# nicklashansen/tdmpc2

Hardware: AMD Instinct MI355X
Metric: plan() calls/sec (H=3, 512 samples, 6 iters) (higher is better)
Workload: dtype f32 (f16x2-split products: 22-bit operands, fp32 accumulate)

## Files before the change

### tdmpc2_amd/csrc/fused_kernels.cuh

```cuda
#pragma once

#include "kloop_schedule.h"

#ifdef SPLIT_TIMING
#define TIMER_FIELDS mutable unsigned long long t_acc[14] = {0, 0, 0, 0, 0, 0, 0, 0, 0, 0, 0, 0, 0, 0}; mutable unsigned long long t_last = 0, t_begin = 0;
#define TIMER_START(c) { (c).t_last = (c).t_begin = __builtin_amdgcn_s_memtime(); }
#define TIMER_MARK(c, cls) { __builtin_amdgcn_sched_barrier(0); const unsigned long long t_now = __builtin_amdgcn_s_memtime(); __builtin_amdgcn_sched_barrier(0); (c).t_acc[cls] += t_now - (c).t_last; (c).t_last = t_now; }
#ifndef SPLIT_TIMING_WAVE
#define SPLIT_TIMING_WAVE 4
#endif
#define TIMER_FLUSH(c, ptr) if ((ptr) && threadIdx.x == 64 * SPLIT_TIMING_WAVE) { for (int i_ = 0; i_ < 14; ++i_) atomicAdd((ptr) + i_, (c).t_acc[i_]); atomicAdd((ptr) + 14, (c).t_last - (c).t_begin); atomicAdd((ptr) + 15, 1ull); }
#else
#define TIMER_FIELDS
#define TIMER_START(c)
#define TIMER_MARK(c, cls)
#define TIMER_FLUSH(c, ptr)
#endif
enum { T_KLOOP = 0, T_EPI = 1, T_HEAD = 2, T_ACT = 3, T_PARK = 4, T_TILE = 5, T_EPI_PRE = 6, T_EPI_SYNC = 7, T_EPI_BIAS = 8,
       T_EPI_COMB = 9, T_EPI_MATH = 10, T_CL_WAIT = 11, T_HEAD_K = 12, T_HEAD_ST = 13 };



template <int APAD, int ST = 2, int NW = 8, int AR = 0>
struct CtxT {
    static constexpr int NST = ST;
    static constexpr int NWAVES = NW;
    static constexpr int ARITH = AR;
    static constexpr int FT = 16 / NW;
    static constexpr int NTHR = 64 * NW;
    static constexpr int TROWS = 32 * ST;
    static constexpr int SH = WIDTH + APAD;
    static constexpr int RSH = 2 * SH + 8;
    static constexpr int RSF_ = AR == 0 ? RSH / 2 : WIDTH + APAD + 4;
    static constexpr int KBLK = AR == 0 ? 16 : 8;
    static constexpr int ZKB = WIDTH / KBLK;
    _Float16 *act;
    float *stats;
    float *gb;
    int tid, wave, lane;
    mutable float pg[(WIDTH + NTHR - 1) / NTHR], pb[(WIDTH + NTHR - 1) / NTHR];
    TIMER_FIELDS
    __device__ __forceinline__ float *f32() const { return reinterpret_cast<float *>(act); }
    static constexpr __device__ __forceinline__ int RSF() { return RSF_; }
};

__device__ __forceinline__ float mish_fast(float x) {
    const float e = __expf(fminf(x, 20.f));
    const float n = e * (e + 2.f);
    return x * (n * __builtin_amdgcn_rcpf(n + 2.f));
}

template <class CT>
__device__ __forceinline__ float exp_a(float x) {
    if constexpr (CT::ARITH == 1) return expf(x);
    else return __expf(x);
}
template <class CT>
__device__ __forceinline__ float mish_a(float x) {
    if constexpr (CT::ARITH == 1) {
        const float e = expf(fminf(x, 20.f));
        const float n = e * (e + 2.f);
        return x * (n / (n + 2.f));
    } else {
        return mish_fast(x);
    }
}

__device__ __forceinline__ void split4(const f32x4 y, f16x4 &hi, f16x4 &lo, const float scale = ACT_SCALE) {
#pragma unroll
    for (int e = 0; e < 4; ++e) {
        const float ys = y[e] * scale;
        const _Float16 h = (_Float16)ys;
        hi[e] = h;
        lo[e] = (_Float16)(ys - (float)h);
    }
}


constexpr int PF = 2;
template <int FT>
struct BFragT {
    f16x8 h[FT], l[FT];
};
__device__ __forceinline__ f16x8 ldw(const char *ubase, unsigned voff, int imm) {
    return *reinterpret_cast<const f16x8 *>(ubase + voff + imm);
}
#define SPLIT_MFMA(a, b, c) __builtin_amdgcn_mfma_f32_32x32x16_f16(a, b, c, 0, 0, 0)
template <int FT>
__device__ __forceinline__ void load_b(BFragT<FT> &b, const char *u0, size_t ct_stride, unsigned voff) {
#pragma unroll
    for (int cc = 0; cc < FT; ++cc) {
        b.h[cc] = ldw(u0 + cc * ct_stride, voff, 0);
        b.l[cc] = ldw(u0 + cc * ct_stride, voff, 1024);
    }
}
template <int ST, int FT>
__device__ __forceinline__ void zero_acc(f32x16 (&a)[ST][FT]) {
#pragma unroll
    for (int r = 0; r < ST; ++r)
#pragma unroll
        for (int cc = 0; cc < FT; ++cc)
#pragma unroll
            for (int e = 0; e < 16; ++e) a[r][cc][e] = 0.f;
}
template <int ST>
struct AFragT {
    f16x8 h[ST], l[ST];
};
template <class CT>
__device__ __forceinline__ void load_a(AFragT<CT::NST> &a, const _Float16 *a0p, int kk) {
#pragma unroll
    for (int st = 0; st < CT::NST; ++st) {
        a.h[st] = *reinterpret_cast<const f16x8 *>(a0p + st * 32 * CT::RSH + kk * 16);
        a.l[st] = *reinterpret_cast<const f16x8 *>(a0p + st * 32 * CT::RSH + CT::SH + kk * 16);
    }
}
template <class CT>
__device__ __forceinline__ void kloop_f32(const CT &c, const LayerS &ly, int kb0, int kb1, f32x16 (&acc)[CT::NST][CT::FT]) {
    constexpr int FT = CT::FT, NST = CT::NST;
    constexpr int PFD = 4;
    const int i = c.lane & 31, hh = c.lane >> 5;
    const float *a0p = c.f32() + i * CT::RSF() + 4 * hh + kb0 * 8;
    const char *u0 = reinterpret_cast<const char *>(ly.wp) + ((size_t)(FT * c.wave) * ly.KB + kb0) * 1024;
    const size_t cts = (size_t)ly.KB * 1024;
    unsigned voff = (unsigned)c.lane * 16u;
    asm volatile("" : "+v"(voff));
// ... 285 lines not shown
        for (int d = 0; d < PFT; ++d) step(k + d, d, true);
    }
#pragma unroll 1
    for (; k < nk; k += PFT) {
#pragma unroll
        for (int d = 0; d < PFT; ++d)
            if (k + d < nk) step(k + d, d, false);
    }
#pragma unroll
    for (int r = 0; r < CT::NST; ++r)
#pragma unroll
        for (int e = 0; e < 16; ++e) out[r][e] = acc[r][0][e] + (acc[r][1][e] + acc[r][2][e]);
}


template <class CT>
__device__ __forceinline__ void park(const CT &c, const f32x16 (&acc)[CT::NST][CT::FT], float *dst) {
#pragma unroll
    for (int st = 0; st < CT::NST; ++st)
#pragma unroll
        for (int ft = 0; ft < CT::FT; ++ft)
#pragma unroll
            for (int m = 0; m < 4; ++m) {
                f32x4 v;
#pragma unroll
                for (int r = 0; r < 4; ++r) v[r] = acc[st][ft][4 * m + r];
                const int idx4 = ((c.wave * CT::NST + st) * CT::FT + ft) * 4 + m;
                *reinterpret_cast<f32x4 *>(dst + ((size_t)idx4 * 64 + c.lane) * 4) = v;
            }
}
template <class CT>
__device__ __forceinline__ void unpark(const CT &c, f32x16 (&acc)[CT::NST][CT::FT], const float *src) {
#pragma unroll
    for (int st = 0; st < CT::NST; ++st)
#pragma unroll
        for (int ft = 0; ft < CT::FT; ++ft)
#pragma unroll
            for (int m = 0; m < 4; ++m) {
                const int idx4 = ((c.wave * CT::NST + st) * CT::FT + ft) * 4 + m;
                const f32x4 v = *reinterpret_cast<const f32x4 *>(src + ((size_t)idx4 * 64 + c.lane) * 4);
#pragma unroll
                for (int r = 0; r < 4; ++r) acc[st][ft][4 * m + r] = v[r];
            }
}

template <class CT>
__device__ __forceinline__ void regs_to_tile(const CT &c, const f32x16 (&y)[CT::NST][CT::FT], const float scale = ACT_SCALE) {
    const int j = c.lane & 31, hh = c.lane >> 5;
    if constexpr (CT::ARITH == 1) {
#pragma unroll
        for (int st = 0; st < CT::NST; ++st) {
            float *fp = c.f32() + (32 * st + j) * CT::RSF() + 32 * CT::FT * c.wave + 4 * hh;
#pragma unroll
            for (int ft = 0; ft < CT::FT; ++ft)
#pragma unroll
                for (int m = 0; m < 4; ++m) {
                    f32x4 v;
#pragma unroll
                    for (int r = 0; r < 4; ++r) v[r] = y[st][ft][4 * m + r];
                    *reinterpret_cast<f32x4 *>(fp + 32 * ft + 8 * m) = v;
                }
        }
        return;
    }
#pragma unroll
    for (int st = 0; st < CT::NST; ++st) {
        _Float16 *hp = c.act + (32 * st + j) * c.RSH + 32 * CT::FT * c.wave + 4 * hh;
#pragma unroll
        for (int ft = 0; ft < CT::FT; ++ft)
#pragma unroll
            for (int m = 0; m < 4; ++m) {
                f32x4 v;
#pragma unroll
                for (int r = 0; r < 4; ++r) v[r] = y[st][ft][4 * m + r];
                f16x4 hi, lo;
                split4(v, hi, lo, scale);
                *reinterpret_cast<f16x4 *>(hp + 32 * ft + 8 * m) = hi;
                *reinterpret_cast<f16x4 *>(hp + c.SH + 32 * ft + 8 * m) = lo;
            }
    }
}

struct GB {
    const float *g = nullptr, *b = nullptr;
};
__device__ __forceinline__ GB gb_of(const LayerS &ly) { return GB{ly.g, ly.b}; }

template <class CT>
__device__ __forceinline__ void gb_prefetch(const CT &c, const float *g, const float *b) {
#pragma unroll
    for (int u = 0; u < (WIDTH + CT::NTHR - 1) / CT::NTHR; ++u) {
        const int f = c.tid + u * CT::NTHR;
        c.pg[u] = f < WIDTH ? g[f] : 0.f;
        c.pb[u] = f < WIDTH ? b[f] : 0.f;
    }
}
template <class CT>
__device__ __forceinline__ void gb_commit(const CT &c) {
#pragma unroll
    for (int u = 0; u < (WIDTH + CT::NTHR - 1) / CT::NTHR; ++u) {
        const int f = c.tid + u * CT::NTHR;
        if (f < WIDTH) {
            c.gb[f] = c.pg[u];
            c.gb[WIDTH + f] = c.pb[u];
        }
    }
}
template <class CT>
__device__ __forceinline__ void epi_barrier(const CT &c) {
    __syncthreads();
    gb_commit(c);
}

enum { EPI_PRE = 1, EPI_MATH = 2, EPI_STORE = 4, EPI_ALL = 7 };
template <int ACT, class CT, bool HASBIAS = true, int PIECES = EPI_ALL>
__device__ __forceinline__ void epi_t(const CT &c, f32x16 (&acc)[CT::NST][CT::FT], float osc, float asc, const float *bias,
                                      GB next, float *zcopy) {
    constexpr int FT = CT::FT, NW = CT::NWAVES;
    constexpr float CNT = 32.f * FT;
    const int j = c.lane & 31, hh = c.lane >> 5;
    const int poff = 32 * FT * c.wave + 4 * hh;
    if constexpr (PIECES & EPI_PRE) {
    if constexpr (HASBIAS) {
#pragma unroll
        for (int ft = 0; ft < FT; ++ft) {
            f32x4 b4[4];
#pragma unroll
            for (int m = 0; m < 4; ++m) b4[m] = *reinterpret_cast<const f32x4 *>(bias + poff + 32 * ft + 8 * m);
#pragma unroll
            for (int m = 0; m < 4; ++m)
#pragma unroll
                for (int st = 0; st < CT::NST; ++st)
#pragma unroll
                    for (int r = 0; r < 4; ++r) acc[st][ft][4 * m + r] = fmaf(acc[st][ft][4 * m + r], osc, b4[m][r]);
        }
    }
    TIMER_MARK(c, T_EPI_BIAS)
#pragma unroll
    for (int st = 0; st < CT::NST; ++st) {
        float s = 0.f;
#pragma unroll
        for (int ft = 0; ft < FT; ++ft)
#pragma unroll
            for (int e = 0; e < 16; ++e) s += acc[st][ft][e];
        s += __shfl_xor(s, 32);
        const float mw = s * (1.0f / CNT);
        float m2 = 0.f;
#pragma unroll
        for (int ft = 0; ft < FT; ++ft)
#pragma unroll
            for (int e = 0; e < 16; ++e) {
                const float d = acc[st][ft][e] - mw;
                m2 = fmaf(d, d, m2);
            }
        m2 += __shfl_xor(m2, 32);
        if (hh == 0) {
            c.stats[(c.wave * CT::TROWS + 32 * st + j) * 2 + 0] = mw;
            c.stats[(c.wave * CT::TROWS + 32 * st + j) * 2 + 1] = m2;
        }
    }
    TIMER_MARK(c, T_EPI_PRE)
    }
    if constexpr (PIECES == EPI_ALL) {
    __syncthreads();
    TIMER_MARK(c, T_EPI_SYNC)
    }
    if constexpr (PIECES & EPI_MATH) {
    float rstd[CT::NST], shift[CT::NST];
#pragma unroll
    for (int st = 0; st < CT::NST; ++st) {
        float pm[NW], mean = 0.f, msum = 0.f;
#pragma unroll
        for (int w = 0; w < NW; ++w) {
            pm[w] = c.stats[(w * CT::TROWS + 32 * st + j) * 2 + 0];
            msum += c.stats[(w * CT::TROWS + 32 * st + j) * 2 + 1];
            mean += pm[w];
        }
        mean *= 1.0f / NW;
#pragma unroll
        for (int w = 0; w < NW; ++w) {
            const float d = pm[w] - mean;
            msum = fmaf(CNT * d, d, msum);
        }
        rstd[st] = 1.0f / sqrtf(msum * (1.0f / WIDTH) + LN_EPS);
        shift[st] = -mean * rstd[st];
    }
    TIMER_MARK(c, T_EPI_COMB)
#pragma unroll
    for (int ft = 0; ft < FT; ++ft) {
        f32x4 gq[4], bq[4];
#pragma unroll
        for (int m = 0; m < 4; ++m) {
            gq[m] = *reinterpret_cast<const f32x4 *>(c.gb + poff + 32 * ft + 8 * m);
            bq[m] = *reinterpret_cast<const f32x4 *>(c.gb + WIDTH + poff + 32 * ft + 8 * m);
        }
#pragma unroll
        for (int m = 0; m < 4; ++m) {
            const f32x4 g4 = gq[m], b4 = bq[m];
#pragma unroll
            for (int st = 0; st < CT::NST; ++st) {
                float y[4];
#pragma unroll
                for (int r = 0; r < 4; ++r) y[r] = fmaf(fmaf(acc[st][ft][4 * m + r], rstd[st], shift[st]), g4[r], b4[r]);
                if (ACT == 0) {
#pragma unroll
                    for (int r = 0; r < 4; ++r) y[r] = mish_a<CT>(y[r]);
                } else {
                    float mx = fmaxf(fmaxf(y[0], y[1]), fmaxf(y[2], y[3]));
                    mx = fmaxf(mx, __shfl_xor(mx, 32));
                    float es = 0.f;
#pragma unroll
// ... 23 lines not shown
    if (zcopy) park(c, acc, zcopy);
    }
}
template <class CT>
__device__ __forceinline__ void epi_pre(const CT &c, f32x16 (&acc)[CT::NST][CT::FT], float osc, const float *bias) {
    epi_t<0, CT, true, EPI_PRE>(c, acc, osc, 0.f, bias, GB{}, nullptr);
}
template <int ACT, class CT>
__device__ __forceinline__ void epi_math(const CT &c, f32x16 (&acc)[CT::NST][CT::FT], float asc) {
    epi_t<ACT, CT, true, EPI_MATH>(c, acc, 0.f, asc, nullptr, GB{}, nullptr);
}
template <int ACT, class CT>
__device__ __forceinline__ void epi_store(const CT &c, f32x16 (&acc)[CT::NST][CT::FT], float asc, float *zcopy) {
    epi_t<ACT, CT, true, EPI_STORE>(c, acc, 0.f, asc, nullptr, GB{}, zcopy);
}

template <class CT>
__device__ __forceinline__ void add_row_bias(const CT &c, f32x16 (&acc)[CT::NST][CT::FT], float osc, const float *const (&brow)[CT::NST]) {
    const int hh = c.lane >> 5;
    const int poff = 32 * CT::FT * c.wave + 4 * hh;
#pragma unroll
    for (int st = 0; st < CT::NST; ++st)
#pragma unroll
        for (int ft = 0; ft < CT::FT; ++ft)
#pragma unroll
            for (int m = 0; m < 4; ++m) {
                const f32x4 b4 = *reinterpret_cast<const f32x4 *>(brow[st] + poff + 32 * ft + 8 * m);
#pragma unroll
                for (int r = 0; r < 4; ++r) acc[st][ft][4 * m + r] = fmaf(acc[st][ft][4 * m + r], osc, b4[r]);
            }
}

template <class CT>
__device__ __forceinline__ void store_tile_s(const CT &c, const f32x16 &acc, float osc, const float *bias, int ct, int rt) {
    float *f = c.f32();
    constexpr int RSF = CT::RSF();
    const int j = c.lane & 31, hh = c.lane >> 5;
    const int col = ct * 32 + j;
    const float bv = bias[col];
#pragma unroll
    for (int reg = 0; reg < 16; ++reg) {
        const int row = rt * 32 + (reg & 3) + 8 * (reg >> 2) + 4 * hh;
        f[row * RSF + col] = fmaf(acc[reg], osc, bv);
    }
}

template <class CT>
__device__ __forceinline__ float twohot_rows_s(const CT &c, const float *bins, int num_bins) {
    const int part = c.tid & 7;
    const bool live = (c.tid >> 3) < CT::TROWS;
    const int row = live ? c.tid >> 3 : 0;
    const float *rp = c.f32() + row * c.RSF();
    if (num_bins <= 1) {
        const float x1 = rp[0];
        return num_bins == 0 ? x1 : symexp_f(x1);
    }
    float v[16];
    float m = -INFINITY;
#pragma unroll
    for (int q = 0; q < 16; ++q) {
        const int jj = part + 8 * q;
        v[q] = (jj < num_bins) ? rp[jj] : -INFINITY;
        m = fmaxf(m, v[q]);
    }
    m = group_max<8>(m);
    float es = 0.f, x = 0.f;
#pragma unroll
    for (int q = 0; q < 16; ++q) {
        const int jj = part + 8 * q;
        const float ev = (jj < num_bins) ? expf(v[q] - m) : 0.f;
        es += ev;
        x = fmaf(ev, (jj < num_bins) ? bins[jj] : 0.f, x);
    }
    es = group_sum<8>(es);
    x = group_sum<8>(x);
    return symexp_f(x / es);
}

template <int ACT, class CT>
__device__ __forceinline__ void layer_full_s(const CT &c, const LayerS &ly, const float *bias, int kb0, int kb1,
                                             GB next, float *zcopy = nullptr) {
    f32x16 acc[CT::NST][CT::FT];
    zero_acc(acc);
    if (next.g) gb_prefetch(c, next.g, next.b);
    kloop_s(c, ly, kb0, kb1, acc);
    TIMER_MARK(c, T_KLOOP)
    epi_t<ACT>(c, acc, *ly.oscale, *ly.ascale, bias, next, zcopy);
    epi_barrier(c);
    TIMER_MARK(c, T_EPI)
}

template <class CT>
__device__ __forceinline__ void head_logits_s(const CT &c, const LayerS &ly) {
    f32x16 acc[CT::NST];
    const float osc = *ly.oscale;
    const int ct = c.wave;
    if (ct < ly.CT) kloop_tile_s(c, ly, ct, 0, CT::ZKB, acc);
    __syncthreads();
    TIMER_MARK(c, T_HEAD_K)
    if (ct < ly.CT) {
#pragma unroll
        for (int rt = 0; rt < CT::NST; ++rt) store_tile_s(c, acc[rt], osc, ly.bias, ct, rt);
    }
    __syncthreads();
    TIMER_MARK(c, T_HEAD_ST)
}

template <class CT>
__device__ __forceinline__ float head_twohot_s(const CT &c, const LayerS &ly, const float *bins, int num_bins) {
    head_logits_s(c, ly);
    const float r = twohot_rows_s(c, bins, num_bins);
    __syncthreads();
    return r;
}

template <class CT>
__device__ __forceinline__ void put_action(const CT &c, int row, int a, float v) {
    if constexpr (CT::ARITH == 1) {
        c.f32()[row * CT::RSF() + WIDTH + a] = v;
        return;
    }
    const float vs = v * ACT_SCALE;
    const _Float16 h = (_Float16)vs;
    _Float16 *rp = c.act + row * c.RSH + WIDTH + a;
    rp[0] = h;
    rp[c.SH] = (_Float16)(vs - (float)h);
}

template <class CT, typename EpsFn>
__device__ __forceinline__ void head_pi_rows_s(const CT &c, int A, int Apad, float lsmin, float lsdif, const float *mask_wg, EpsFn eps,
                                               float *gdst, int nvalid, float *tsc, const float *mask_tab = nullptr,
                                               const int *row_task = nullptr, int put_rows = CT::TROWS, bool agent_store = false);

template <class CT, typename EpsFn>
__device__ __forceinline__ void head_pi_s(const CT &c, const LayerS &ly, int A, int Apad, float lsmin, float lsdif,
                                          const float *mask_wg, EpsFn eps, float *gdst, int nvalid, float *tsc,
                                          const float *mask_tab = nullptr, const int *row_task = nullptr) {
    head_logits_s(c, ly);
    head_pi_rows_s(c, A, Apad, lsmin, lsdif, mask_wg, eps, gdst, nvalid, tsc, mask_tab, row_task, CT::TROWS, false);
}

template <class CT, typename EpsFn>
__device__ __forceinline__ void head_pi_rows_s(const CT &c, int A, int Apad, float lsmin, float lsdif, const float *mask_wg, EpsFn eps,
                                               float *gdst, int nvalid, float *tsc, const float *mask_tab, const int *row_task,
                                               int put_rows, bool agent_store) {
    const int row = c.tid >> 3, part = c.tid & 7;
    const float *rp = c.f32() + row * c.RSF();
    const float *mask = mask_wg;
    if (mask_tab && row < CT::TROWS) mask = mask_tab + (size_t)row_task[row] * A;
    if (row < CT::TROWS)
    for (int a = part; a < Apad; a += 8) {
        float out = 0.f;
        if (a < A) {
            float mu = rp[a], lsr = rp[A + a];
            float ls = lsmin + 0.5f * lsdif * (tanhf(lsr) + 1.f);
            float e = eps(row, a);
            if (mask) {
                const float mk = mask[a];
                mu *= mk;
                ls *= mk;
                e *= mk;
            }
            out = tanhf(mu + e * expf(ls));
            if (gdst && row < nvalid) {
                if (agent_store) __hip_atomic_store(gdst + row * A + a, out, __ATOMIC_RELAXED, __HIP_MEMORY_SCOPE_AGENT);
                else gdst[row * A + a] = out;
            }
            if (tsc) tsc[a] = out;
        }
        if (row < put_rows) put_action(c, row, a, out);
// ... 154 lines not shown
                  p.actions + ((size_t)e * p.H + t) * p.N * p.A, p.P, nullptr);
        if (t == p.H - 1) break;
        tile_from_global_s(c, zs);
        __syncthreads();
        layer_full_s<0>(c, p.dyn.l[0], b_dyn, 0, KBA, gb_of(p.dyn.l[1]));
        layer_full_s<0>(c, p.dyn.l[1], p.dyn.l[1].bias, 0, ZKB16, gb_of(p.dyn.l[2]));
        layer_full_s<1>(c, p.dyn.l[2], p.dyn.l[2].bias, 0, ZKB16, gb_of(p.pi.l[0]), zs);
    }
}

template <class CT>
__device__ __forceinline__ float head_term_s(const CT &c, const LayerS &ly) {
    f32x16 acc[CT::NST];
    if (c.wave == 0) kloop_tile_s(c, ly, 0, 0, CT::ZKB, acc);
    const float osc = *ly.oscale;
    __syncthreads();
    if (c.wave == 0) {
#pragma unroll
        for (int rt = 0; rt < CT::NST; ++rt) store_tile_s(c, acc[rt], osc, ly.bias, 0, rt);
    }
    __syncthreads();
    const bool live = (c.tid >> 3) < CT::TROWS;
    const float x = c.f32()[(live ? c.tid >> 3 : 0) * c.RSF()];
    const float pr = 1.f / (1.f + expf(-x));
    __syncthreads();
    return pr > 0.5f ? 1.f : 0.f;
}

template <class CT>
__device__ __forceinline__ void first_layers_s(const CT &c, const LayerS &la, const LayerS &lb, int kb0, int kb1,
                                               f32x16 (&acca)[CT::NST][CT::FT], f32x16 (&accb)[CT::NST][CT::FT]) {
    zero_acc(acca);
    zero_acc(accb);
    kloop_s(c, la, kb0, kb1, acca);
    kloop_s(c, lb, kb0, kb1, accb);
}

template <class CT>
__device__ __forceinline__ void sample_actions(const CT &c, const RolloutParams &p, const int e, const int row0, const float *mask,
                                               const float *sm_mean, const float *sm_std, const int t) {
    constexpr int TROWS = CT::TROWS, NTHR = CT::NTHR;
    const int tid = c.tid;
    float *ag = p.actions + ((size_t)e * p.H + t) * p.N * p.A;
    const int hp = p.Apad / 2;
    for (int idx = tid; idx < TROWS * hp; idx += NTHR) {
        const int row = idx / hp, a0 = 2 * (idx % hp);
        const int n = row0 + row;
        float v[2] = {0.f, 0.f};
        const bool sampled = !(p.given_actions || n < p.P);
        float z[2] = {0.f, 0.f};
        if (sampled && a0 < p.A && !p.sample_eps) {
            const unsigned pair = (unsigned)(((size_t)t * (p.N - p.P) + (n - p.P)) * hp + a0 / 2);
            rng_normal2(p.seed, p.call, SITE_SAMPLE, p.iter, e, pair, z[0], z[1]);
        }
#pragma unroll
        for (int u = 0; u < 2; ++u) {
            const int a = a0 + u;
            if (a < p.A) {
                if (!sampled) {
                    v[u] = ag[(size_t)n * p.A + a];
                } else {
                    float r = z[u];
                    if (p.sample_eps)
                        r = p.sample_eps[(size_t)e * p.sample_eps_estride +
                                         (unsigned)(((size_t)t * (p.N - p.P) + (n - p.P)) * p.A + a)];
                    v[u] = sample_action(sm_mean[t * p.A + a], sm_std[t * p.A + a], r);
                }
                if (mask && !p.given_actions) v[u] *= mask[a];
                if (!p.given_actions) ag[(size_t)n * p.A + a] = v[u];
            }
            put_action(c, row, a, v[u]);
        }
    }
}

#define DUMP_TILE(...) do { if constexpr (TRACE) dump_tile_s(__VA_ARGS__); } while (0)
template <int APAD, int ST, int NW, int AR, int EP, int TR = 0>
__global__ __launch_bounds__(64 * NW, 2) void ks_rollout(RolloutParams p) {
    constexpr bool TRACE = TR || EP;
    extern __shared__ __attribute__((aligned(16))) float smem[];
    __shared__ int s_is_last;
    const int e = blockIdx.x / p.tiles, tile = p.tile_off + blockIdx.x % p.tiles;
    const int tid = threadIdx.x;
    typedef CtxT<APAD, ST, NW, AR> CT;
    constexpr int TROWS = CT::TROWS, NTHR = CT::NTHR, FT = CT::FT;
    constexpr int ZKB16 = CT::ZKB;
    CT c{reinterpret_cast<_Float16 *>(smem), smem + TROWS * CT::RSF(), smem + TROWS * CT::RSF() + 1024, tid,
         __builtin_amdgcn_readfirstlane(tid >> 6), tid & 63};
    float *sm_mean = smem + TROWS * CT::RSF() + 2048;
    float *sm_std = sm_mean + p.H * p.A;
    const int row0 = tile * TROWS;
    const float *mask = p.act_mask ? p.act_mask + (size_t)e * p.A : nullptr;
    const float *disc = p.disc_pow + (size_t)e * (p.H + 1);
    const int KBA = ZKB16 + p.Apad / CT::KBLK;
    float *zs = p.zscratch + (size_t)blockIdx.x * TROWS * WIDTH;
    const int NSLOT = 5 * p.H + 7;
    const bool live = (tid >> 3) < TROWS;
    float *tsc = nullptr;
    if constexpr (TRACE) tsc = p.trace_scalars && live ? p.trace_scalars + ((size_t)e * p.N + row0 + (tid >> 3)) * (p.H + 2 + p.A) : nullptr;

    for (int idx = tid; idx < p.H * p.A; idx += NTHR) {
        sm_mean[idx] = p.mean[(size_t)e * p.H * p.A + idx];
        sm_std[idx] = p.std[(size_t)e * p.H * p.A + idx];
    }
    int q0, q1;
    if (p.qidx) {
        q0 = p.qidx[(size_t)e * p.qidx_estride + 0];
        q1 = p.qidx[(size_t)e * p.qidx_estride + 1];
    } else {
        const uint4 r = rng_raw(p.seed, p.call, SITE_QIDX, p.iter, e, 0);
        q0 = (int)(r.x % (unsigned)p.nq);
        q1 = (int)(r.y % (unsigned)(p.nq - 1));
        if (q1 >= q0) ++q1;
    }
    const float *b_rew = p.multitask ? p.beff + ((size_t)e * p.nnets + BE_REW) * WIDTH : p.rew.l[0].bias;
    const float *b_dyn = p.multitask ? p.beff + ((size_t)e * p.nnets + BE_DYN) * WIDTH : p.dyn.l[0].bias;
    const float *b_pi = p.multitask ? p.beff + ((size_t)e * p.nnets + BE_PI) * WIDTH : p.pi.l[0].bias;
    const float *b_q0 = p.multitask ? p.beff + ((size_t)e * p.nnets + BE_Q0 + q0) * WIDTH : p.q[q0].l[0].bias;
    const float *b_q1 = p.multitask ? p.beff + ((size_t)e * p.nnets + BE_Q0 + q1) * WIDTH : p.q[q1].l[0].bias;
    gb_prefetch(c, p.rew.l[0].g, p.rew.l[0].b);
    epi_barrier(c);

    float G = 0.f;
    float termv = 0.f;
    TIMER_START(c)
    for (int t = 0; t < p.H; ++t) {
        sample_actions(c, p, e, row0, mask, sm_mean, sm_std, t);
        __syncthreads();
        TIMER_MARK(c, T_ACT)
        const bool term_step = EP && t > 0;
        f32x16 accd[ST][FT];
        {
            f32x16 acc[ST][FT];
            gb_prefetch(c, p.rew.l[1].g, p.rew.l[1].b);
            first_layers_s(c, p.dyn.l[0], p.rew.l[0], t == 0 ? ZKB16 : 0, KBA, accd, acc);
            TIMER_MARK(c, T_KLOOP)
            if constexpr (EP) {
                if (term_step) {
                    park(c, accd, zs);
                    zero_acc(accd);
                    kloop_s(c, p.term.l[0], 0, ZKB16, accd);
                }
            }
            epi_t<0>(c, acc, *p.rew.l[0].oscale, *p.rew.l[0].ascale, t == 0 ? p.cvec + ((size_t)e * 2 + 0) * WIDTH : b_rew,
                     gb_of(p.rew.l[1]), nullptr);
        }
        epi_barrier(c);
        TIMER_MARK(c, T_EPI)
        DUMP_TILE(c, p.trace_tiles, NSLOT, 5 * t + 0, p.rew.l[0].ascale);
        layer_full_s<0>(c, p.rew.l[1], p.rew.l[1].bias, 0, ZKB16, term_step ? gb_of(p.term.l[0]) : gb_of(p.dyn.l[0]));
        DUMP_TILE(c, p.trace_tiles, NSLOT, 5 * t + 1, p.rew.l[1].ascale);
        if (term_step) gb_prefetch(c, p.term.l[1].g, p.term.l[1].b);
        else gb_prefetch(c, p.dyn.l[1].g, p.dyn.l[1].b);
        const float r = head_twohot_s(c, p.rew.l[2], p.bins, p.num_bins);
        TIMER_MARK(c, T_HEAD)
        if (tsc && (tid & 7) == 0) tsc[t] = r;
        if constexpr (EP) {
            if (term_step) {
                epi_t<0>(c, accd, *p.term.l[0].oscale, *p.term.l[0].ascale, p.term.l[0].bias, gb_of(p.term.l[1]), nullptr);
                epi_barrier(c);
                layer_full_s<0>(c, p.term.l[1], p.term.l[1].bias, 0, ZKB16, gb_of(p.dyn.l[0]));
                gb_prefetch(c, p.dyn.l[1].g, p.dyn.l[1].b);
                termv = fminf(termv + head_term_s(c, p.term.l[2]), 1.f);
                unpark(c, accd, zs);
            }
        }
        G += disc[t] * (1.f - termv) * r;
        epi_t<0>(c, accd, *p.dyn.l[0].oscale, *p.dyn.l[0].ascale, t == 0 ? p.cvec + ((size_t)e * 2 + 1) * WIDTH : b_dyn,
                 gb_of(p.dyn.l[1]), nullptr);
        epi_barrier(c);
        TIMER_MARK(c, T_EPI)
        DUMP_TILE(c, p.trace_tiles, NSLOT, 5 * t + 2, p.dyn.l[0].ascale);
        layer_full_s<0>(c, p.dyn.l[1], p.dyn.l[1].bias, 0, ZKB16, gb_of(p.dyn.l[2]));
        DUMP_TILE(c, p.trace_tiles, NSLOT, 5 * t + 3, p.dyn.l[1].ascale);
        layer_full_s<1>(c, p.dyn.l[2], p.dyn.l[2].bias, 0, ZKB16, t == p.H - 1 ? gb_of(p.pi.l[0]) : gb_of(p.rew.l[0]),
                        t == p.H - 1 ? zs : nullptr);
        DUMP_TILE(c, p.trace_tiles, NSLOT, 5 * t + 4);
    }
    f32x16 acch[ST][FT];
    if constexpr (EP) {
        zero_acc(acch);
        kloop_s(c, p.term.l[0], 0, ZKB16, acch);
    }
    layer_full_s<0>(c, p.pi.l[0], b_pi, 0, ZKB16, gb_of(p.pi.l[1]));
    DUMP_TILE(c, p.trace_tiles, NSLOT, 5 * p.H + 0, p.pi.l[0].ascale);
    layer_full_s<0>(c, p.pi.l[1], p.pi.l[1].bias, 0, ZKB16, EP ? gb_of(p.term.l[0]) : gb_of(p.q[q0].l[0]));
    DUMP_TILE(c, p.trace_tiles, NSLOT, 5 * p.H + 1, p.pi.l[1].ascale);
    if constexpr (EP) gb_prefetch(c, p.term.l[1].g, p.term.l[1].b);
    {
        auto eps = [&](int row, int a) -> float {
            const unsigned ridx = (unsigned)((size_t)(row0 + row) * p.A + a);
            if (p.pi_eps) return p.pi_eps[(size_t)e * p.pi_eps_estride + ridx];
            return rng_normal(p.seed, p.call, SITE_PI, p.iter, e, ridx);
        };
        head_pi_s(c, p.pi.l[2], p.A, p.Apad, p.log_std_min, p.log_std_dif, mask, eps, nullptr, 0,
                  tsc ? tsc + p.H + 2 : nullptr);
    }
    TIMER_MARK(c, T_HEAD)
    if constexpr (EP) {
        epi_t<0>(c, acch, *p.term.l[0].oscale, *p.term.l[0].ascale, p.term.l[0].bias, gb_of(p.term.l[1]), nullptr);
        epi_barrier(c);
        layer_full_s<0>(c, p.term.l[1], p.term.l[1].bias, 0, ZKB16, gb_of(p.q[q0].l[0]));
        termv = fminf(termv + head_term_s(c, p.term.l[2]), 1.f);
    }
    tile_from_global_s(c, zs);
    __syncthreads();
    TIMER_MARK(c, T_TILE)
    DUMP_TILE(c, p.trace_tiles, NSLOT, 5 * p.H + 2);
    {
        f32x16 acc[ST][FT];
        gb_prefetch(c, p.q[q0].l[1].g, p.q[q0].l[1].b);
        first_layers_s(c, p.q[q1].l[0], p.q[q0].l[0], 0, KBA, acch, acc);
        TIMER_MARK(c, T_KLOOP)
        epi_t<0>(c, acc, *p.q[q0].l[0].oscale, *p.q[q0].l[0].ascale, b_q0, gb_of(p.q[q0].l[1]), nullptr);
    }
    epi_barrier(c);
    TIMER_MARK(c, T_EPI)
    DUMP_TILE(c, p.trace_tiles, NSLOT, 5 * p.H + 3, p.q[q0].l[0].ascale);
    layer_full_s<0>(c, p.q[q0].l[1], p.q[q0].l[1].bias, 0, ZKB16, gb_of(p.q[q1].l[0]));
    DUMP_TILE(c, p.trace_tiles, NSLOT, 5 * p.H + 4, p.q[q0].l[1].ascale);
    gb_prefetch(c, p.q[q1].l[1].g, p.q[q1].l[1].b);
    const float qa = head_twohot_s(c, p.q[q0].l[2], p.bins, p.num_bins);
    TIMER_MARK(c, T_HEAD)
    epi_t<0>(c, acch, *p.q[q1].l[0].oscale, *p.q[q1].l[0].ascale, b_q1, gb_of(p.q[q1].l[1]), nullptr);
    epi_barrier(c);
    TIMER_MARK(c, T_EPI)
    DUMP_TILE(c, p.trace_tiles, NSLOT, 5 * p.H + 5, p.q[q1].l[0].ascale);
    layer_full_s<0>(c, p.q[q1].l[1], p.q[q1].l[1].bias, 0, ZKB16, GB{});
    DUMP_TILE(c, p.trace_tiles, NSLOT, 5 * p.H + 6, p.q[q1].l[1].ascale);
    const float qb = head_twohot_s(c, p.q[q1].l[2], p.bins, p.num_bins);
    TIMER_MARK(c, T_HEAD)
    TIMER_FLUSH(c, p.timing)
    if (tsc && (tid & 7) == 0) {
        tsc[p.H] = qa;
        tsc[p.H + 1] = qb;
    }
    const float val = G + disc[p.H] * (1.f - termv) * ((qa + qb) / 2.f);
    if (!p.fold_refit) {
        if ((tid & 7) == 0 && live) p.value[(size_t)e * p.N + row0 + (tid >> 3)] = val;
        return;
    }
    if ((tid & 7) == 0 && live)
        __hip_atomic_store(p.value + (size_t)e * p.N + row0 + (tid >> 3), val, __ATOMIC_RELAXED, __HIP_MEMORY_SCOPE_AGENT);
    asm volatile("s_waitcnt vmcnt(0)" ::: "memory");
    __builtin_amdgcn_fence(__ATOMIC_RELEASE, "workgroup");
    __syncthreads();
    if (tid == 0) {
        const unsigned old = __hip_atomic_fetch_add(p.ticket + e, 1u, __ATOMIC_RELAXED, __HIP_MEMORY_SCOPE_AGENT);
        const int last = old == (unsigned)(p.tiles - 1);
        if (last) __hip_atomic_store(p.ticket + e, 0u, __ATOMIC_RELAXED, __HIP_MEMORY_SCOPE_AGENT);
        s_is_last = last;
    }
    __syncthreads();
    if (!s_is_last) return;
    refit_plan(p.rf, e, smem, tid, NTHR);
}

template <int APAD, int AR>
__global__ __launch_bounds__(NTHREADS, 2) void ks_value(ValueParams p) {
    extern __shared__ __attribute__((aligned(16))) float smem[];
    const int tid = threadIdx.x;
    typedef CtxT<APAD, 2, 8, AR> CT;
    constexpr int TROWS = CT::TROWS, ZKB16 = CT::ZKB;
    CT c{reinterpret_cast<_Float16 *>(smem), smem + TROWS * CT::RSF(), smem + TROWS * CT::RSF() + 1024, tid,
         __builtin_amdgcn_readfirstlane(tid >> 6), tid & 63};
    int *s_task = reinterpret_cast<int *>(smem + TROWS * CT::RSF() + 2048);
    const int row0 = blockIdx.x * TROWS;
    const int nvalid = min(TROWS, p.rows - row0);
    const float *zsrc = p.z + (size_t)row0 * WIDTH;
    const int KBA = ZKB16 + p.Apad / CT::KBLK;
    int q0, q1;
    if (p.qidx) {
        q0 = p.qidx[0];
        q1 = p.qidx[1];
    } else {
        const uint4 r = rng_raw(p.seed, p.call, SITE_QIDX, 0, 0, 0);
        q0 = (int)(r.x % (unsigned)p.nq);
        q1 = (int)(r.y % (unsigned)(p.nq - 1));
        if (q1 >= q0) ++q1;
    }
    if (p.task_ids && tid < TROWS) s_task[tid] = tid < nvalid ? p.task_ids[row0 + tid] : 0;
    tile_from_rows_s(c, zsrc, nvalid);
    gb_prefetch(c, p.pi.l[0].g, p.pi.l[0].b);
    epi_barrier(c);
    const int j = c.lane & 31;
    auto first_layer = [&](const LayerS &ly, int slot, int kb1, GB next) {
        if (!p.task_ids) {
            layer_full_s<0>(c, ly, ly.bias, 0, kb1, next);
            return;
        }
        const float *brow[CT::NST];
#pragma unroll
        for (int st = 0; st < CT::NST; ++st) brow[st] = p.beff_tab + ((size_t)s_task[32 * st + j] * p.nnets + slot) * WIDTH;
        f32x16 acc[CT::NST][CT::FT];
        zero_acc(acc);
        if (next.g) gb_prefetch(c, next.g, next.b);
        kloop_s(c, ly, 0, kb1, acc);
        add_row_bias(c, acc, *ly.oscale, brow);
        epi_t<0, CT, false>(c, acc, 1.f, *ly.ascale, nullptr, next, nullptr);
        epi_barrier(c);
    };
    first_layer(p.pi.l[0], BE_PI, ZKB16, gb_of(p.pi.l[1]));
    layer_full_s<0>(c, p.pi.l[1], p.pi.l[1].bias, 0, ZKB16, gb_of(p.q[q0].l[0]));
    {
// ... 30 lines not shown
```

Baseline: 9865.

## Stage next-layer bias through LDS and keep final latent in registers

Adds a per-thread bias prefetch alongside the gamma/beta prefetch. At the epilogue barrier the bias is committed into the stats LDS region, so the bias-add reads LDS instead of global memory. Separately, in the non-episodic path the last dynamics layer's output is held in accumulator registers and written straight into the activation tile, replacing the global write and reload of zs. This trades global traffic and latency for extra register pressure and reuse of LDS scratch, which could hurt occupancy or collide with stats usage.

Result: faster. 10030, median of 6 (+1.6%).

```diff
diff --git a/tdmpc2_amd/csrc/fused_kernels.cuh b/tdmpc2_amd/csrc/fused_kernels.cuh
--- a/tdmpc2_amd/csrc/fused_kernels.cuh
+++ b/tdmpc2_amd/csrc/fused_kernels.cuh
@@ -21,8 +21,19 @@
 
 
 
+#ifdef KS_NO_BIAS_LDS
+constexpr bool KS_BIAS_LDS = false;
+#else
+constexpr bool KS_BIAS_LDS = true;
+#endif
+#ifdef KS_NO_ZH_REGS
+constexpr bool KS_ZH_REGS = false;
+#else
+constexpr bool KS_ZH_REGS = true;
+#endif
 template <int APAD, int ST = 2, int NW = 8, int AR = 0>
 struct CtxT {
+    static constexpr bool BIAS_LDS = false;
     static constexpr int NST = ST;
     static constexpr int NWAVES = NW;
     static constexpr int ARITH = AR;
@@ -42,6 +53,11 @@
     TIMER_FIELDS
     __device__ __forceinline__ float *f32() const { return reinterpret_cast<float *>(act); }
     static constexpr __device__ __forceinline__ int RSF() { return RSF_; }
+};
+template <int APAD, int ST, int NW, int AR>
+struct CtxPhT : CtxT<APAD, ST, NW, AR> {
+    static constexpr bool BIAS_LDS = KS_BIAS_LDS;
+    mutable float pbias = 0.f;
 };
 
 __device__ __forceinline__ float mish_fast(float x) {
@@ -493,9 +509,10 @@
 }
 
 struct GB {
-    const float *g = nullptr, *b = nullptr;
+    const float *g = nullptr, *b = nullptr, *bias = nullptr;
 };
-__device__ __forceinline__ GB gb_of(const LayerS &ly) { return GB{ly.g, ly.b}; }
+__device__ __forceinline__ GB gb_of(const LayerS &ly) { return GB{ly.g, ly.b, ly.bias}; }
+__device__ __forceinline__ GB gb_of(const LayerS &ly, const float *bias) { return GB{ly.g, ly.b, bias}; }
 
 template <class CT>
 __device__ __forceinline__ void gb_prefetch(const CT &c, const float *g, const float *b) {
@@ -507,7 +524,16 @@
     }
 }
 template <class CT>
+__device__ __forceinline__ void gb_prefetch(const CT &c, const GB next) {
+    gb_prefetch(c, next.g, next.b);
+    if constexpr (CT::BIAS_LDS) {
+        static_assert(CT::FT == 2 && CT::NTHR == WIDTH, "thread tid fetches feature tid of its own wave's 64");
+        c.pbias = next.bias[c.tid];
+    }
+}
+template <class CT>
 __device__ __forceinline__ void gb_commit(const CT &c) {
+    if constexpr (CT::BIAS_LDS) c.stats[c.wave * (CT::TROWS * 2) + c.lane] = c.pbias;
 #pragma unroll
     for (int u = 0; u < (WIDTH + CT::NTHR - 1) / CT::NTHR; ++u) {
         const int f = c.tid + u * CT::NTHR;
@@ -537,7 +563,11 @@
         for (int ft = 0; ft < FT; ++ft) {
             f32x4 b4[4];
 #pragma unroll
-            for (int m = 0; m < 4; ++m) b4[m] = *reinterpret_cast<const f32x4 *>(bias + poff + 32 * ft + 8 * m);
+            for (int m = 0; m < 4; ++m) {
+                if constexpr (CT::BIAS_LDS)
+                    b4[m] = *reinterpret_cast<const f32x4 *>(c.stats + c.wave * (CT::TROWS * 2) + 4 * hh + 32 * ft + 8 * m);
+                else b4[m] = *reinterpret_cast<const f32x4 *>(bias + poff + 32 * ft + 8 * m);
+            }
 #pragma unroll
             for (int m = 0; m < 4; ++m)
 #pragma unroll
@@ -727,10 +757,21 @@
                                              GB next, float *zcopy = nullptr) {
     f32x16 acc[CT::NST][CT::FT];
     zero_acc(acc);
-    if (next.g) gb_prefetch(c, next.g, next.b);
+    if (next.g) gb_prefetch(c, next);
     kloop_s(c, ly, kb0, kb1, acc);
     TIMER_MARK(c, T_KLOOP)
     epi_t<ACT>(c, acc, *ly.oscale, *ly.ascale, bias, next, zcopy);
+    epi_barrier(c);
+    TIMER_MARK(c, T_EPI)
+}
+template <int ACT, class CT>
+__device__ __forceinline__ void layer_held_s(const CT &c, const LayerS &ly, const float *bias, int kb0, int kb1, GB next,
+                                             f32x16 (&acc)[CT::NST][CT::FT]) {
+    zero_acc(acc);
+    if (next.g) gb_prefetch(c, next);
+    kloop_s(c, ly, kb0, kb1, acc);
+    TIMER_MARK(c, T_KLOOP)
+    epi_t<ACT>(c, acc, *ly.oscale, *ly.ascale, bias, next, nullptr);
     epi_barrier(c);
     TIMER_MARK(c, T_EPI)
 }
@@ -1051,11 +1092,12 @@
     __shared__ int s_is_last;
     const int e = blockIdx.x / p.tiles, tile = p.tile_off + blockIdx.x % p.tiles;
     const int tid = threadIdx.x;
-    typedef CtxT<APAD, ST, NW, AR> CT;
+    typedef CtxPhT<APAD, ST, NW, AR> CT;
     constexpr int TROWS = CT::TROWS, NTHR = CT::NTHR, FT = CT::FT;
     constexpr int ZKB16 = CT::ZKB;
-    CT c{reinterpret_cast<_Float16 *>(smem), smem + TROWS * CT::RSF(), smem + TROWS * CT::RSF() + 1024, tid,
-         __builtin_amdgcn_readfirstlane(tid >> 6), tid & 63};
+    constexpr bool ZH_REGS = !EP && KS_ZH_REGS;
+    CT c{{reinterpret_cast<_Float16 *>(smem), smem + TROWS * CT::RSF(), smem + TROWS * CT::RSF() + 1024, tid,
+          __builtin_amdgcn_readfirstlane(tid >> 6), tid & 63}};
     float *sm_mean = smem + TROWS * CT::RSF() + 2048;
     float *sm_std = sm_mean + p.H * p.A;
     const int row0 = tile * TROWS;
@@ -1087,7 +1129,8 @@
     const float *b_pi = p.multitask ? p.beff + ((size_t)e * p.nnets + BE_PI) * WIDTH : p.pi.l[0].bias;
     const float *b_q0 = p.multitask ? p.beff + ((size_t)e * p.nnets + BE_Q0 + q0) * WIDTH : p.q[q0].l[0].bias;
     const float *b_q1 = p.multitask ? p.beff + ((size_t)e * p.nnets + BE_Q0 + q1) * WIDTH : p.q[q1].l[0].bias;
-    gb_prefetch(c, p.rew.l[0].g, p.rew.l[0].b);
+    const float *c_rew = p.cvec + ((size_t)e * 2 + 0) * WIDTH, *c_dyn = p.cvec + ((size_t)e * 2 + 1) * WIDTH;
+    gb_prefetch(c, gb_of(p.rew.l[0], c_rew));
     epi_barrier(c);
 
     float G = 0.f;
@@ -1101,7 +1144,7 @@
         f32x16 accd[ST][FT];
         {
             f32x16 acc[ST][FT];
-            gb_prefetch(c, p.rew.l[1].g, p.rew.l[1].b);
+            gb_prefetch(c, gb_of(p.rew.l[1]));
             first_layers_s(c, p.dyn.l[0], p.rew.l[0], t == 0 ? ZKB16 : 0, KBA, accd, acc);
             TIMER_MARK(c, T_KLOOP)
             if constexpr (EP) {
@@ -1111,16 +1154,16 @@
                     kloop_s(c, p.term.l[0], 0, ZKB16, accd);
                 }
             }
-            epi_t<0>(c, acc, *p.rew.l[0].oscale, *p.rew.l[0].ascale, t == 0 ? p.cvec + ((size_t)e * 2 + 0) * WIDTH : b_rew,
-                     gb_of(p.rew.l[1]), nullptr);
+            epi_t<0>(c, acc, *p.rew.l[0].oscale, *p.rew.l[0].ascale, t == 0 ? c_rew : b_rew, gb_of(p.rew.l[1]), nullptr);
         }
         epi_barrier(c);
         TIMER_MARK(c, T_EPI)
         DUMP_TILE(c, p.trace_tiles, NSLOT, 5 * t + 0, p.rew.l[0].ascale);
-        layer_full_s<0>(c, p.rew.l[1], p.rew.l[1].bias, 0, ZKB16, term_step ? gb_of(p.term.l[0]) : gb_of(p.dyn.l[0]));
+        layer_full_s<0>(c, p.rew.l[1], p.rew.l[1].bias, 0, ZKB16,
+                        term_step ? gb_of(p.term.l[0]) : gb_of(p.dyn.l[0], t == 0 ? c_dyn : b_dyn));
         DUMP_TILE(c, p.trace_tiles, NSLOT, 5 * t + 1, p.rew.l[1].ascale);
-        if (term_step) gb_prefetch(c, p.term.l[1].g, p.term.l[1].b);
-        else gb_prefetch(c, p.dyn.l[1].g, p.dyn.l[1].b);
+        if (term_step) gb_prefetch(c, gb_of(p.term.l[1]));
+        else gb_prefetch(c, gb_of(p.dyn.l[1]));
         const float r = head_twohot_s(c, p.rew.l[2], p.bins, p.num_bins);
         TIMER_MARK(c, T_HEAD)
         if (tsc && (tid & 7) == 0) tsc[t] = r;
@@ -1128,34 +1171,42 @@
             if (term_step) {
                 epi_t<0>(c, accd, *p.term.l[0].oscale, *p.term.l[0].ascale, p.term.l[0].bias, gb_of(p.term.l[1]), nullptr);
                 epi_barrier(c);
-                layer_full_s<0>(c, p.term.l[1], p.term.l[1].bias, 0, ZKB16, gb_of(p.dyn.l[0]));
-                gb_prefetch(c, p.dyn.l[1].g, p.dyn.l[1].b);
+                layer_full_s<0>(c, p.term.l[1], p.term.l[1].bias, 0, ZKB16, gb_of(p.dyn.l[0], b_dyn));
+                gb_prefetch(c, gb_of(p.dyn.l[1]));
                 termv = fminf(termv + head_term_s(c, p.term.l[2]), 1.f);
                 unpark(c, accd, zs);
             }
         }
         G += disc[t] * (1.f - termv) * r;
-        epi_t<0>(c, accd, *p.dyn.l[0].oscale, *p.dyn.l[0].ascale, t == 0 ? p.cvec + ((size_t)e * 2 + 1) * WIDTH : b_dyn,
-                 gb_of(p.dyn.l[1]), nullptr);
+        epi_t<0>(c, accd, *p.dyn.l[0].oscale, *p.dyn.l[0].ascale, t == 0 ? c_dyn : b_dyn, gb_of(p.dyn.l[1]), nullptr);
         epi_barrier(c);
         TIMER_MARK(c, T_EPI)
         DUMP_TILE(c, p.trace_tiles, NSLOT, 5 * t + 2, p.dyn.l[0].ascale);
         layer_full_s<0>(c, p.dyn.l[1], p.dyn.l[1].bias, 0, ZKB16, gb_of(p.dyn.l[2]));
         DUMP_TILE(c, p.trace_tiles, NSLOT, 5 * t + 3, p.dyn.l[1].ascale);
-        layer_full_s<1>(c, p.dyn.l[2], p.dyn.l[2].bias, 0, ZKB16, t == p.H - 1 ? gb_of(p.pi.l[0]) : gb_of(p.rew.l[0]),
-                        t == p.H - 1 ? zs : nullptr);
+        if constexpr (ZH_REGS) {
+            if (t == p.H - 1) break;
+            layer_full_s<1>(c, p.dyn.l[2], p.dyn.l[2].bias, 0, ZKB16, gb_of(p.rew.l[0], b_rew), nullptr);
+        } else {
+            layer_full_s<1>(c, p.dyn.l[2], p.dyn.l[2].bias, 0, ZKB16,
+                            t == p.H - 1 ? gb_of(p.pi.l[0], b_pi) : gb_of(p.rew.l[0], b_rew), t == p.H - 1 ? zs : nullptr);
+        }
         DUMP_TILE(c, p.trace_tiles, NSLOT, 5 * t + 4);
     }
     f32x16 acch[ST][FT];
+    if constexpr (ZH_REGS) {
+        layer_held_s<1>(c, p.dyn.l[2], p.dyn.l[2].bias, 0, ZKB16, gb_of(p.pi.l[0], b_pi), acch);
+        DUMP_TILE(c, p.trace_tiles, NSLOT, 5 * (p.H - 1) + 4);
+    }
     if constexpr (EP) {
         zero_acc(acch);
         kloop_s(c, p.term.l[0], 0, ZKB16, acch);
     }
     layer_full_s<0>(c, p.pi.l[0], b_pi, 0, ZKB16, gb_of(p.pi.l[1]));
     DUMP_TILE(c, p.trace_tiles, NSLOT, 5 * p.H + 0, p.pi.l[0].ascale);
-    layer_full_s<0>(c, p.pi.l[1], p.pi.l[1].bias, 0, ZKB16, EP ? gb_of(p.term.l[0]) : gb_of(p.q[q0].l[0]));
+    layer_full_s<0>(c, p.pi.l[1], p.pi.l[1].bias, 0, ZKB16, EP ? gb_of(p.term.l[0]) : gb_of(p.q[q0].l[0], b_q0));
     DUMP_TILE(c, p.trace_tiles, NSLOT, 5 * p.H + 1, p.pi.l[1].ascale);
-    if constexpr (EP) gb_prefetch(c, p.term.l[1].g, p.term.l[1].b);
+    if constexpr (EP) gb_prefetch(c, gb_of(p.term.l[1]));
     {
         auto eps = [&](int row, int a) -> float {
             const unsigned ridx = (unsigned)((size_t)(row0 + row) * p.A + a);
@@ -1169,16 +1220,17 @@
     if constexpr (EP) {
         epi_t<0>(c, acch, *p.term.l[0].oscale, *p.term.l[0].ascale, p.term.l[0].bias, gb_of(p.term.l[1]), nullptr);
         epi_barrier(c);
-        layer_full_s<0>(c, p.term.l[1], p.term.l[1].bias, 0, ZKB16, gb_of(p.q[q0].l[0]));
+        layer_full_s<0>(c, p.term.l[1], p.term.l[1].bias, 0, ZKB16, gb_of(p.q[q0].l[0], b_q0));
         termv = fminf(termv + head_term_s(c, p.term.l[2]), 1.f);
     }
-    tile_from_global_s(c, zs);
+    if constexpr (ZH_REGS) regs_to_tile(c, acch);
+    else tile_from_global_s(c, zs);
     __syncthreads();
     TIMER_MARK(c, T_TILE)
     DUMP_TILE(c, p.trace_tiles, NSLOT, 5 * p.H + 2);
     {
         f32x16 acc[ST][FT];
-        gb_prefetch(c, p.q[q0].l[1].g, p.q[q0].l[1].b);
+        gb_prefetch(c, gb_of(p.q[q0].l[1]));
         first_layers_s(c, p.q[q1].l[0], p.q[q0].l[0], 0, KBA, acch, acc);
         TIMER_MARK(c, T_KLOOP)
         epi_t<0>(c, acc, *p.q[q0].l[0].oscale, *p.q[q0].l[0].ascale, b_q0, gb_of(p.q[q0].l[1]), nullptr);
@@ -1186,9 +1238,9 @@
     epi_barrier(c);
     TIMER_MARK(c, T_EPI)
     DUMP_TILE(c, p.trace_tiles, NSLOT, 5 * p.H + 3, p.q[q0].l[0].ascale);
-    layer_full_s<0>(c, p.q[q0].l[1], p.q[q0].l[1].bias, 0, ZKB16, gb_of(p.q[q1].l[0]));
+    layer_full_s<0>(c, p.q[q0].l[1], p.q[q0].l[1].bias, 0, ZKB16, gb_of(p.q[q1].l[0], b_q1));
     DUMP_TILE(c, p.trace_tiles, NSLOT, 5 * p.H + 4, p.q[q0].l[1].ascale);
-    gb_prefetch(c, p.q[q1].l[1].g, p.q[q1].l[1].b);
+    gb_prefetch(c, gb_of(p.q[q1].l[1]));
     const float qa = head_twohot_s(c, p.q[q0].l[2], p.bins, p.num_bins);
     TIMER_MARK(c, T_HEAD)
     epi_t<0>(c, acch, *p.q[q1].l[0].oscale, *p.q[q1].l[0].ascale, b_q1, gb_of(p.q[q1].l[1]), nullptr);
```
